# ohjay/snn-modulation-classification

Hardware: AMD Instinct MI355X
Metric: IQ windows/sec (RadioML 2x128, T=128) (higher is better)
Workload: dtype f32

## Files before the change

snn_modulation_classification_amd/csrc/dcll_hip.hip:

```cpp
#include "dcll_internal.h"

static thread_local char g_err[DCLL_ERR_LEN] = "";
char *dcll_err_buf(void) { return g_err; }

extern "C" int dcll_version(void) { return DCLL_ABI_VERSION; }
extern "C" const char *dcll_last_error(void) { return g_err; }

constexpr size_t DCLL_TRACE_LEN = 1 << 16;
static thread_local bool g_trace_on = false;
static thread_local size_t g_trace_len = 0;
static thread_local char *g_trace = nullptr;
void dcll_trace_note(const char *name)
{
    if (!g_trace_on || !g_trace) return;
    const size_t n = strlen(name);
    if (g_trace_len + n + 5 >= DCLL_TRACE_LEN) {
        if (g_trace_len + 4 < DCLL_TRACE_LEN && (g_trace_len < 4 || memcmp(g_trace + g_trace_len - 4, "...\n", 4) != 0)) {
            memcpy(g_trace + g_trace_len, "...\n", 4);
            g_trace_len += 4;
        }
        return;
    }
    memcpy(g_trace + g_trace_len, name, n);
    g_trace[g_trace_len + n] = '\n';
// ... 1251 lines not shown
            if (NRO > 0) {
                constexpr int RO_CH = (NRO > 24) ? 6 : 12;
                const f32x4 *wp = (const f32x4 *)ro_Wp + (long)((me * 4 + wq) * NRO) * 64 + lane;
#pragma unroll
                for (int n0 = 0; n0 < NRO; n0 += RO_CH) {
                    f32x4 wb[RO_CH];
#pragma unroll
                    for (int k = 0; k < RO_CH; ++k) wb[k] = wp[(n0 + k) * 64];
                    __builtin_amdgcn_sched_barrier(0);
#pragma unroll
                    for (int k = 0; k < RO_CH; ++k)
                        racc[n0 + k] = __builtin_fmaf(pvq[0], wb[k][0], __builtin_fmaf(pvq[1], wb[k][1],
                                       __builtin_fmaf(pvq[2], wb[k][2], __builtin_fmaf(pvq[3], wb[k][3], racc[n0 + k]))));
                    __builtin_amdgcn_sched_barrier(0);
                }
                if ((me >> 1) == 3) {
                    float *dst = ropart + ((te & 1) * NWAVE + w) * NRO;
#pragma unroll
                    for (int n = 0; n < NRO; ++n) {
                        const float tot = wave_sum_to_lane63(racc[n]);
                        if (lane == 63) dst[n] = tot;
                        racc[n] = 0.0f;
                    }
                }
            }
        }
        if (NRO > 0) {
            const int gc = g - 16;
            if (gc >= 0 && (gc & 7) == 0 && (gc >> 3) < T && w == ((gc >> 3) & 7) && lane < NRO) {
                const int tc = gc >> 3;
                const float *src = ropart + ((tc & 1) * NWAVE) * NRO + lane;
                float tot = ro_b[lane];
#pragma unroll
                for (int k = 0; k < NWAVE; ++k) tot += src[k * NRO];
                ro_out[((long)tc * B + b) * NRO + lane] = tot;
            }
        }
        if (ABLATE & 8) { unsigned long long x_ = __builtin_amdgcn_s_memtime(); dbg_epi += x_ - dbg_a; dbg_a = x_; }
        const int q = g - w;
        const bool active = q >= 0 && q < 8 * T;
        const bool tracing = active && !(ABLATE & 2) && (((q & 7) & 1) == tpar) && (q >> 3) + 1 < T;
        if (loaded && !tracing && !(PRIO & 4)) __builtin_amdgcn_s_setprio(0);
        if (active) {
            const int m = q & 7, t = q >> 3;
            float *img = lds + (t & 1) * IMG_FLOATS;
            if (tracing) {
                const int c = m >> 1;
                const float ta = tau4[0 * 32 + 4 * w + c], tm = tau4[1 * 32 + 4 * w + c];
                const float tas = tau4[2 * 32 + 4 * w + c], ts = tau4[3 * 32 + 4 * w + c];
                const unsigned long long w0 = pw0, w1 = pw1, w2 = pw2, w3 = pw3;
                {
                    const int tn = (c < 3) ? t + 1 : t + 2, cn = (c + 1) & 3;
                    if (tn < T) {
                        const unsigned long long *ip = in_wave + (long)tn * in_step + cn * 4;
                        pw0 = ip[0]; pw1 = ip[1]; pw2 = ip[2]; pw3 = ip[3];
                    }
                }
                const float *src = img + ioff + c * CHF;
                float *dst = lds + ((t + 1) & 1) * IMG_FLOATS + ioff + c * CHF;
                const float s0 = src[0], s1 = src[4 * ROWF], s2 = src[8 * ROWF], s3 = src[12 * ROWF];
                switch (c) {
#define DCLL_TRACE_CASE(C)                                                                \
    case C:                                                                               \
        trace_elem(w0, e0[C * 4 + 0], s0, dst + 0 * 4 * ROWF, ta, tm, tas, ts);           \
        trace_elem(w1, e0[C * 4 + 1], s1, dst + 1 * 4 * ROWF, ta, tm, tas, ts);           \
        trace_elem(w2, e0[C * 4 + 2], s2, dst + 2 * 4 * ROWF, ta, tm, tas, ts);           \
        trace_elem(w3, e0[C * 4 + 3], s3, dst + 3 * 4 * ROWF, ta, tm, tas, ts);           \
        break;
                    DCLL_TRACE_CASE(0)
                    DCLL_TRACE_CASE(1)
                    DCLL_TRACE_CASE(2)
                    DCLL_TRACE_CASE(3)
#undef DCLL_TRACE_CASE
                }
            }
            if (ABLATE & 8) { unsigned long long x_ = __builtin_amdgcn_s_memtime(); dbg_tr += x_ - dbg_a; dbg_a = x_; }
            if (loaded && tracing && !(PRIO & 4)) __builtin_amdgcn_s_setprio(0);
            f32x16 acc;
            if (w == 0 || (ABLATE & 4)) {
#pragma unroll
                for (int r = 0; r < 16; ++r) acc[r] = sbias[(r & 3) + 8 * (r >> 2) + 4 * h];
            } else {
                const f32x4 *sp = (const f32x4 *)(slots + ((w - 1) * 2 + ((g - 1) & 1)) * SLOT_FLOATS) + lane;
#pragma unroll
                for (int c = 0; c < 4; ++c) {
                    f32x4 v4 = sp[c * 64];
                    acc[4 * c + 0] = v4[0]; acc[4 * c + 1] = v4[1]; acc[4 * c + 2] = v4[2]; acc[4 * c + 3] = v4[3];
                }
            }
            const int i0 = (t & 1) * IMG_FLOATS + bbase + m * 2 * ROWF;
            int i1 = i0 + 2 * CHF;
            if (BASES == 2) asm volatile("" : "+v"(i1));
            auto tapval = [&](int cp, int off) -> float { return (BASES == 2 && cp) ? lds[i1 + off] : lds[i0 + cp * 2 * CHF + off]; };
            float bq[2][7];
#pragma unroll
            for (int kx = 0; kx < 7; ++kx) bq[0][kx] = tapval(0, kx);
#pragma unroll
            for (int r = 0; r < 14; ++r) {
                if (r + 1 < 14) {
                    const int cpn = (r + 1) / 7, kyn = (r + 1) % 7;
#pragma unroll
                    for (int kx = 0; kx < 7; ++kx) bq[(r + 1) & 1][kx] = tapval(cpn, kyn * ROWF + kx);
                }
                __builtin_amdgcn_sched_barrier(0);
#pragma unroll
                for (int kx = 0; kx < 7; ++kx)
                    acc = __builtin_amdgcn_mfma_f32_32x32x2f32(wf[r / 7][(r % 7) * 7 + kx], bq[r & 1][kx], acc, 0, 0, 0);
                __builtin_amdgcn_sched_barrier(0);
            }
            f32x4 *dp = (f32x4 *)(slots + (w * 2 + (g & 1)) * SLOT_FLOATS) + lane;
            if (ABLATE & 4) {
                if (acc[0] + acc[5] + acc[10] + acc[15] == 12345.678f) dp[0] = f32x4{acc[0], acc[1], acc[2], acc[3]};
            } else {
#pragma unroll
                for (int c = 0; c < 4; ++c) {
                    f32x4 v4 = {acc[4 * c + 0], acc[4 * c + 1], acc[4 * c + 2], acc[4 * c + 3]};
                    dp[c * 64] = v4;
                }
            }
        }
        if (loaded && (PRIO & 4)) __builtin_amdgcn_s_setprio(0);
        if (ABLATE & 8) {
            asm volatile("s_waitcnt vmcnt(0) lgkmcnt(0)" ::: "memory");
            unsigned long long x_ = __builtin_amdgcn_s_memtime();
            dbg_mf += x_ - dbg_a;
            __syncthreads();
            dbg_wait += __builtin_amdgcn_s_memtime() - x_;
        } else {
            __syncthreads();
        }
    }
    if ((ABLATE & 8) && lane == 0 && b == 0) {
        unsigned long long tot = __builtin_amdgcn_s_memtime() - dbg_t0;
        unsigned long long *dp = (unsigned long long *)v_out + w * 8;
        dp[0] = tot; dp[1] = dbg_wait; dp[2] = dbg_epi; dp[3] = dbg_tr; dp[4] = dbg_mf;
    }

    const float *fin = lds + ((T - 1) & 1) * IMG_FLOATS;
#pragma unroll
    for (int i = 0; i < 16; ++i) {
        long gidx = (b * 32 + 4 * w + (i >> 2)) * 256 + (i & 3) * 64 + lane;
        eps0_g[gidx] = e0[i];
        eps1_g[gidx] = fin[ioff + (i >> 2) * CHF + (i & 3) * 4 * ROWF];
    }
    if (REFRACTORY) {
#pragma unroll
        for (int k = 0; k < 4; ++k)
#pragma unroll
            for (int rr = 0; rr < 4; ++rr)
                arp_g[(b * 32 + rr + 8 * wq + 4 * h) * 256 + 32 * (2 * k + wpar) + j] = arp[k][rr];
    }
}

template <bool REFRACTORY, int OUT, int DBG = 0>
__global__ __launch_bounds__(512) void k_lif_seq_c32d(const uint32_t *__restrict__ spk_in, const dcll_wsrc W,
                                                       const float *__restrict__ bias, const float *__restrict__ tau4,
                                                       float *__restrict__ eps0_g, float *__restrict__ eps1_g,
                                                       float *__restrict__ arp_g, uint32_t *__restrict__ spk_out,
                                                       float *__restrict__ pv_out, float *__restrict__ v_out, int T,
                                                       int B, float alpharp, float wrp)
{
    __shared__ __attribute__((aligned(16))) float lds[2 * IMG_FLOATS + (NWAVE * 2 + 1) * SLOT_FLOATS];
    float *slots = lds + 2 * IMG_FLOATS;
    float *sbias = slots + NWAVE * 2 * SLOT_FLOATS;
    const int tid = threadIdx.x, lane = tid & 63, h = lane >> 5, j = lane & 31;
    const int wi = __builtin_amdgcn_readfirstlane(tid >> 6);
    const int w = (DBG & 4) ? wi : ((wi & 1) | ((wi & 4) >> 1) | ((wi & 2) << 1));
    const int wq = w & 3, wpar = w >> 2;
    const long b = blockIdx.x;
    __builtin_amdgcn_s_setprio(3);

    for (int i = tid; i < 2 * IMG_FLOATS; i += 512) lds[i] = 0.0f;
    for (int i = tid; i < SLOT_FLOATS; i += 512) sbias[i] = bias[(i & 3) + 8 * (i >> 8) + 4 * ((i >> 7) & 1)];

    float wf[2][49];
    load_wf_c32(W, j, w, h, wf);

    float e0[4][4];
    const int ioff = (4 * w) * CHF + ((lane >> 4) + 3) * ROWF + (lane & 15) + 3;
    const unsigned long long *in_wave = (const unsigned long long *)(spk_in + (b * 32 + 4 * w) * 8);
    const long in_step = (long)B * 32 * 4;
    __syncthreads();

#pragma unroll
    for (int grp = 0; grp < 4; ++grp) {
        const int c = (grp - w) & 3;
        const float ta = tau4[0 * 32 + 4 * w + c], tm = tau4[1 * 32 + 4 * w + c];
        const float tas = tau4[2 * 32 + 4 * w + c], ts = tau4[3 * 32 + 4 * w + c];
#pragma unroll
        for (int ii = 0; ii < 4; ++ii) {
            const long gidx = (b * 32 + 4 * w + c) * 256 + ii * 64 + lane;
            e0[grp][ii] = eps0_g[gidx];
            float e1 = eps1_g[gidx];
            float xin = (float)((in_wave[c * 4 + ii] >> lane) & 1ull);
            trace_update(xin, ta, tm, tas, ts, e0[grp][ii], e1);
            lds[ioff + c * CHF + ii * 4 * ROWF] = e1;
        }
    }
    float arp[4][4];
#pragma unroll
    for (int k = 0; k < 4; ++k)
#pragma unroll
        for (int rr = 0; rr < 4; ++rr)
            arp[k][rr] = REFRACTORY ? arp_g[(b * 32 + rr + 8 * wq + 4 * h) * 256 + 32 * (2 * k + wpar) + j] : 0.0f;

    const int bbase = (4 * w + h) * CHF + (j >> 4) * ((DBG & 2) ? 16 : ROWF) + (j & 15);
    const unsigned eoff = 4u * (4 * h * 256 + 32 * wpar + j);
#pragma unroll
    for (int k = 0; k < 4; ++k)
#pragma unroll
        for (int rr = 0; rr < 4; ++rr) asm volatile("" ::"v"(arp[k][rr]));
#pragma unroll
    for (int grp = 0; grp < 4; ++grp)
#pragma unroll
        for (int ii = 0; ii < 4; ++ii) asm volatile("" ::"v"(e0[grp][ii]));
#pragma unroll
    for (int cp = 0; cp < 2; ++cp)
#pragma unroll
        for (int k = 0; k < 49; ++k) asm volatile("" ::"v"(wf[cp][k]));
    __syncthreads();

    unsigned long long dbg[4] = {0, 0, 0, 0}, dbg_t0 = 0;
    if (DBG & 1) dbg_t0 = __builtin_amdgcn_s_memtime();
    float sv[4] = {0.f, 0.f, 0.f, 0.f}, ta = 0.f, tm = 0.f, tas = 0.f, ts = 0.f;
    unsigned long long wm[4] = {0, 0, 0, 0};
    auto fetch_trace_inputs = [&](const int g) {
        const int q = g - w;
        if (q >= 0 && q < 4 * T && (q >> 2) + 1 < T) {
            const int p = q & 3, t = q >> 2;
            const float *src = lds + (t & 1) * IMG_FLOATS + ioff + p * CHF;
#pragma unroll
            for (int i = 0; i < 4; ++i) sv[i] = src[i * 4 * ROWF];
            const unsigned long long *ip = in_wave + (long)(t + 1) * in_step + p * 4;
#pragma unroll
            for (int i = 0; i < 4; ++i) wm[i] = ip[i];
            ta = tau4[0 * 32 + 4 * w + p]; tm = tau4[1 * 32 + 4 * w + p];
            tas = tau4[2 * 32 + 4 * w + p]; ts = tau4[3 * 32 + 4 * w + p];
        }
    };
    fetch_trace_inputs(0);
    auto stage = [&](const int g, auto UC) {
        constexpr int U = decltype(UC)::value;
        unsigned long long st0 = 0, st1 = 0, st2 = 0, st3 = 0;
        if (DBG & 1) st0 = __builtin_amdgcn_s_memtime();
        const int q = g - w;
        const bool active = q >= 0 && q < 4 * T;
        const int p = q & 3, t = q >> 2;
        f32x16 accA, accB;
        if (active) {
            const float *inA = (w == 0) ? sbias : slots + ((w - 1) * 2) * SLOT_FLOATS;
            const float *inB = (w == 0) ? sbias : slots + ((w - 1) * 2 + 1) * SLOT_FLOATS;
            const f32x4 *spa = (const f32x4 *)inA + lane, *spb = (const f32x4 *)inB + lane;
#pragma unroll
            for (int c = 0; c < 4; ++c) {
                f32x4 va = spa[c * 64], vb = spb[c * 64];
                accA[4 * c + 0] = va[0]; accA[4 * c + 1] = va[1]; accA[4 * c + 2] = va[2]; accA[4 * c + 3] = va[3];
                accB[4 * c + 0] = vb[0]; accB[4 * c + 1] = vb[1]; accB[4 * c + 2] = vb[2]; accB[4 * c + 3] = vb[3];
            }
        }
        const int qe = g - 8;
        const bool epi = qe >= 0 && qe < 4 * T;
        f32x4 v4 = {0.f, 0.f, 0.f, 0.f};
        if (epi) v4 = *((const f32x4 *)(slots + (7 * 2 + wpar) * SLOT_FLOATS) + wq * 64 + lane);
        const bool tr = active && t + 1 < T;
        const int i0 = (t & 1) * IMG_FLOATS + bbase + p * 4 * ROWF;
        const bool skip = !(DBG & 4);
        const int rl = (skip && p == 0) ? 2 : 0;
        lds_cfloat *ib0 = (lds_cfloat *)(lds + i0), *ib1 = (lds_cfloat *)(lds + i0 + 2 * CHF);
        asm volatile("" : "+v"(ib0), "+v"(ib1));
        float bq[2][7];
        if (active) {
#pragma unroll
            for (int kx = 0; kx < 7; ++kx) bq[0][kx] = ib0[rl * ROWF + kx];
        }
        if (tr) {
            float *dst = lds + ((t + 1) & 1) * IMG_FLOATS + ioff + p * CHF;
#pragma unroll
            for (int i = 0; i < 4; ++i) {
                float a;
                asm("v_cndmask_b32 %0, 0, %1, %2" : "=v"(a) : "v"(ts), "s"(wm[i]));
                const float bb = tas * e0[U][i];
                e0[U][i] = a + bb;
                const float cc = ta * sv[i];
                const float dd = e0[U][i] * tm;
                dst[i * 4 * ROWF] = cc + dd;
            }
        }
        if (epi) {
            const int te = qe >> 2, me = 2 * U + wpar;
            const long ubase = (((long)te * B + b) * 32 + 8 * wq) * 256;
            const auto prs = tile_rsrc(pv_out + ubase), vrs = tile_rsrc(v_out + ubase);
            uint32_t myword = 0;
#pragma unroll
            for (int rr = 0; rr < 4; ++rr) {
                float v = v4[rr];
                bool s;
                if (REFRACTORY) v = refractory(v4[rr], arp[U][rr], alpharp, wrp, s);
                else s = v > 0.0f;
                const unsigned long long mk = __ballot(s);
                const uint32_t mine = h ? (uint32_t)(mk >> 32) : (uint32_t)mk;
                myword = (j == rr) ? mine : myword;
                if (OUT & 1) __builtin_amdgcn_raw_buffer_store_b32(__float_as_uint(sigmoidf_dev(v)), prs, eoff + 4u * (rr * 256 + 64 * U), 0, 0);
                if (OUT & 2) __builtin_amdgcn_raw_buffer_store_b32(__float_as_uint(v), vrs, eoff + 4u * (rr * 256 + 64 * U), 0, 0);
            }
            if (spk_out && j < 4)
                __builtin_amdgcn_raw_buffer_store_b32(myword, tile_rsrc(spk_out + (ubase >> 5)), 4u * ((4 * h + j) * 8 + wpar) + 8u * U, 0, 0);
        }
        if (DBG & 1) { asm volatile("s_waitcnt lgkmcnt(0)" ::: "memory"); st1 = __builtin_amdgcn_s_memtime(); }
        lds_barrier();
        if (DBG & 1) st2 = __builtin_amdgcn_s_memtime();
        fetch_trace_inputs(g + 1);
        if (active) {
            auto chains = [&](auto RLC, auto RHC) {
                constexpr int RL = decltype(RLC)::value, RH = decltype(RHC)::value, NRH = RH - RL, NR = 2 * NRH;
#pragma unroll
                for (int r = 0; r < NR; ++r) {
                    const int cp = r / NRH, rho = RL + r % NRH;
                    if (r + 1 < NR) {
                        const int cpn = (r + 1) / NRH, rhon = RL + (r + 1) % NRH;
#pragma unroll
                        for (int kx = 0; kx < 7; ++kx) bq[(r + 1) & 1][kx] = (cpn ? ib1 : ib0)[rhon * ROWF + kx];
                    }
                    __builtin_amdgcn_sched_barrier(0);
#pragma unroll
                    for (int kx = 0; kx < 7; ++kx) {
                        if (rho <= 6)
                            accA = __builtin_amdgcn_mfma_f32_32x32x2f32(wf[cp][rho * 7 + kx], bq[r & 1][kx], accA, 0, 0, 0);
                        if (rho >= 2)
                            accB = __builtin_amdgcn_mfma_f32_32x32x2f32(wf[cp][(rho - 2) * 7 + kx], bq[r & 1][kx], accB, 0, 0, 0);
                    }
                    __builtin_amdgcn_sched_barrier(0);
                    if (cp == 1 && rho == 6 && r + 1 < NR) {
                        f32x4 *dpa = (f32x4 *)(slots + (w * 2) * SLOT_FLOATS) + lane;
#pragma unroll
                        for (int c = 0; c < 4; ++c)
                            dpa[c * 64] = f32x4{accA[4 * c + 0], accA[4 * c + 1], accA[4 * c + 2], accA[4 * c + 3]};
                        __builtin_amdgcn_sched_barrier(0);
                    }
                }
                if (RH == 7) {
                    f32x4 *dpa = (f32x4 *)(slots + (w * 2) * SLOT_FLOATS) + lane;
#pragma unroll
                    for (int c = 0; c < 4; ++c)
                        dpa[c * 64] = f32x4{accA[4 * c + 0], accA[4 * c + 1], accA[4 * c + 2], accA[4 * c + 3]};
                }
            };
            if (skip && p == 0) chains(std::integral_constant<int, 2>{}, std::integral_constant<int, 9>{});
            else if (skip && p == 3) chains(std::integral_constant<int, 0>{}, std::integral_constant<int, 7>{});
            else chains(std::integral_constant<int, 0>{}, std::integral_constant<int, 9>{});
            f32x4 *dp = (f32x4 *)(slots + (w * 2 + 1) * SLOT_FLOATS) + lane;
#pragma unroll
            for (int c = 0; c < 4; ++c)
                dp[c * 64] = f32x4{accB[4 * c + 0], accB[4 * c + 1], accB[4 * c + 2], accB[4 * c + 3]};
        }
        if (DBG & 1) { asm volatile("s_waitcnt lgkmcnt(0)" ::: "memory"); st3 = __builtin_amdgcn_s_memtime(); }
        lds_barrier();
        if (DBG & 1) {
            const unsigned long long st4 = __builtin_amdgcn_s_memtime();
            dbg[0] += st1 - st0; dbg[1] += st2 - st1; dbg[2] += st3 - st2; dbg[3] += st4 - st3;
        }
    };

    const int nstage = 4 * T + 8;
    for (int g = 0; g < nstage; g += 4) {
        stage(g + 0, std::integral_constant<int, 0>{});
        stage(g + 1, std::integral_constant<int, 1>{});
        stage(g + 2, std::integral_constant<int, 2>{});
        stage(g + 3, std::integral_constant<int, 3>{});
    }

    if ((DBG & 1) && lane == 0 && b == 0) {
        unsigned long long *dp = (unsigned long long *)v_out + w * 8;
        dp[0] = __builtin_amdgcn_s_memtime() - dbg_t0;
        dp[1] = dbg[0]; dp[2] = dbg[1]; dp[3] = dbg[2]; dp[4] = dbg[3];
    }
    const float *fin = lds + ((T - 1) & 1) * IMG_FLOATS;
#pragma unroll
    for (int grp = 0; grp < 4; ++grp) {
        const int c = (grp - w) & 3;
#pragma unroll
        for (int ii = 0; ii < 4; ++ii) {
            const long gidx = (b * 32 + 4 * w + c) * 256 + ii * 64 + lane;
            eps0_g[gidx] = e0[grp][ii];
            eps1_g[gidx] = fin[ioff + c * CHF + ii * 4 * ROWF];
        }
    }
    if (REFRACTORY) {
#pragma unroll
        for (int k = 0; k < 4; ++k)
#pragma unroll
            for (int rr = 0; rr < 4; ++rr)
                arp_g[(b * 32 + rr + 8 * wq + 4 * h) * 256 + 32 * (2 * k + wpar) + j] = arp[k][rr];
    }
}

__global__ void k_permute_readout(const float *__restrict__ Wt, float *__restrict__ Wp, int N)
{
    int i = blockIdx.x * blockDim.x + threadIdx.x;
    if (i >= N * 8192) return;
    int rr = i & 3, lane = (i >> 2) & 63;
    int r = i >> 8;
    int n = r % N;
    r /= N;
    int wq = r & 3, me = r >> 2;
    int co = rr + 8 * wq + 4 * (lane >> 5), pix = 32 * me + (lane & 31);
    Wp[i] = Wt[(long)n * 8192 + co * 256 + pix];
}

static inline unsigned nblk(long n, int bs) { return (unsigned)((n + bs - 1) / bs); }

static int launch_readout(const float *pv, const float *Wt, const float *bias, float *out, long rows, int K, int N,
                          hipStream_t st, int mode = DCLL_READOUT_AUTO)
{
    if (rows == 0 || N == 0) return DCLL_OK;
    const bool fast = (K % RO_KC == 0) && N <= 64 && (((uintptr_t)pv | (uintptr_t)Wt) & 15) == 0 &&
                      K < (1 << 22);
    const bool direct_ok = fast && K % 64 == 0 && N <= 48 && K <= 16384 && mode != DCLL_READOUT_LDS;
    if (direct_ok && mode == DCLL_READOUT_CORESIDENT)
        return dcll_launch_readout_direct(pv, Wt, bias, out, rows, K, N, st);
    if (fast && mode == DCLL_READOUT_T16) return dcll_launch_readout_t16(pv, Wt, bias, out, rows, K, N, 0, st);
    if (rows <= 2048) {
        hipLaunchKernelGGL(k_readout_rows, dim3((unsigned)((rows + RS_RB - 1) / RS_RB), (N + RS_NG - 1) / RS_NG), dim3(256),
                           0, st, pv, Wt, bias, out, rows, K, N);
    } else if (fast && K % RK_KC == 0 && K >= 65536 && rows < 256L * RO_ROWS) {
        if (N <= 32)
            hipLaunchKernelGGL(k_readout_ks<1>, dim3(nblk(rows, RK_ROWS)), dim3(256), 0, st, pv, Wt, bias, out, rows, K, N, 0);
        else
            hipLaunchKernelGGL(k_readout_ks<2>, dim3(nblk(rows, RK_ROWS)), dim3(256), 0, st, pv, Wt, bias, out, rows, K, N, 0);
    } else if (fast && mode != DCLL_READOUT_LDS) {
        return dcll_launch_readout_t16(pv, Wt, bias, out, rows, K, N, 0, st);
    } else if (fast && N <= 32) {
        hipLaunchKernelGGL(k_readout_v4<1>, dim3(nblk(rows, RO_ROWS)), dim3(256), 0, st, pv, Wt, bias, out, rows, K, N);
    } else if (fast) {
        hipLaunchKernelGGL(k_readout_v4<2>, dim3(nblk(rows, RO_ROWS)), dim3(256), 0, st, pv, Wt, bias, out, rows, K, N);
    } else {
        dim3 grid(nblk(rows, RO_ROWS), (N + 31) / 32);
        hipLaunchKernelGGL(k_readout, grid, dim3(256), 0, st, pv, Wt, bias, out, rows, K, N);
    }
    HIP_CHECK_LAUNCH("k_readout");
    return DCLL_OK;
}

extern "C" int dcll_readout(const float *pv, const float *Wt, const float *bias, float *out, int64_t rows, int32_t K,
                            int32_t N, void *stream)
{
    if (rows == 0) return DCLL_OK;
    if (!pv || !Wt || !out || rows < 0 || K < 1 || N < 1) return fail(DCLL_ERR_INVALID, "dcll_readout: bad argument");
    return launch_readout(pv, Wt, bias, out, rows, K, N, (hipStream_t)stream);
}

extern "C" int dcll_readout_mode(const float *pv, const float *Wt, const float *bias, float *out, int64_t rows,
                                 int32_t K, int32_t N, int32_t mode, void *stream)
{
    if (rows == 0) return DCLL_OK;
    if (!pv || !Wt || !out || rows < 0 || K < 1 || N < 1 || mode < DCLL_READOUT_AUTO || mode > DCLL_READOUT_T16)
        return fail(DCLL_ERR_INVALID, "dcll_readout_mode: bad argument");
    return launch_readout(pv, Wt, bias, out, rows, K, N, (hipStream_t)stream, mode);
}

__global__ __launch_bounds__(256) void k_readout_sum(const float *__restrict__ part, const float *__restrict__ bias,
                                                      float *__restrict__ out, long n_out, int N, int nslice)
{
    __shared__ float red[4][64];
    const long i = (long)blockIdx.x * 64 + (threadIdx.x & 63);
    const int grp = threadIdx.x >> 6;
    float acc = 0.0f;
    if (i < n_out) {
        const int per = (nslice + 3) / 4, s0 = grp * per, s1 = min(nslice, s0 + per);
        for (int sl = s0; sl < s1; ++sl) acc += part[(long)sl * n_out + i];
    }
    red[grp][threadIdx.x & 63] = acc;
    __syncthreads();
    if (grp == 0 && i < n_out) {
        const int l = threadIdx.x & 63;
        out[i] = (bias ? bias[i % N] : 0.0f) + (((red[0][l] + red[1][l]) + red[2][l]) + red[3][l]);
    }
}

static int splitk_slice(int64_t rows, int32_t K, int32_t N)
{
    if (rows < 1 || N < 1 || N > 64) return 0;
    if (K >= 65536 && K % 4096 == 0) {
        return rows <= 2048 ? 4096 : K / 8;
    }
    if (rows <= 2048 && K >= 2048 && K < 65536 && K % 256 == 0) return (rows <= 512 && N <= 32) ? 128 : 256;
    return 0;
}

extern "C" int64_t dcll_readout_splitk_scratch(int64_t rows, int32_t K, int32_t N)
{
    const int ks = splitk_slice(rows, K, N);
    return ks ? (int64_t)(K / ks) * rows * N : 0;
}

extern "C" int dcll_readout_splitk(const float *pv, const float *Wt, const float *bias, float *out, float *scratch,
                                   int64_t scratch_floats, int64_t rows, int32_t K, int32_t N, void *stream)
{
    if (rows == 0 || N == 0) return DCLL_OK;
    if (!pv || !Wt || !out || !scratch || rows < 0 || K < 1 || N < 1)
        return fail(DCLL_ERR_INVALID, "dcll_readout_splitk: bad argument");
    const int ks = splitk_slice(rows, K, N);
    if (ks == 0 || ((((uintptr_t)pv | (uintptr_t)Wt)) & 15) != 0)
        return fail(DCLL_ERR_UNSUPPORTED, "dcll_readout_splitk: needs N <= 64, 16-byte aligned operands and K >= 65536 with "
                                          "K % 4096 == 0, or rows <= 2048 with 2048 <= K < 65536, K % 256 == 0");
    if (scratch_floats < dcll_readout_splitk_scratch(rows, K, N))
        return fail(DCLL_ERR_INVALID, "dcll_readout_splitk: scratch too small (dcll_readout_splitk_scratch)");
    hipStream_t st = (hipStream_t)stream;
    const int nslice = K / ks;
    if (ks != 4096) {
        int rc = dcll_launch_readout_t16(pv, Wt, nullptr, scratch, rows, K, N, ks, st);
        if (rc) return rc;
    } else {
        dim3 grid(nblk(rows, RK_ROWS), nslice);
        if (N <= 32) hipLaunchKernelGGL(k_readout_ks<1>, grid, dim3(256), 0, st, pv, Wt, bias, scratch, rows, K, N, 4096);
        else hipLaunchKernelGGL(k_readout_ks<2>, grid, dim3(256), 0, st, pv, Wt, bias, scratch, rows, K, N, 4096);
        HIP_CHECK_LAUNCH("k_readout_ks (split K)");
    }
    hipLaunchKernelGGL(k_readout_sum, dim3(nblk(rows * N, 64)), dim3(256), 0, st, scratch, bias, out, rows * N, N, nslice);
    HIP_CHECK_LAUNCH("k_readout_sum");
    return DCLL_OK;
}

static int act_nslice(int32_t K)
{
    if (K < 65536 || K % 256 != 0) return 0;
    int n = 8;
    while (n < 64 && K / (2 * n) >= 8192 && K % (2 * n * RO_KC) == 0) n *= 2;
    return n;
}
extern "C" int64_t dcll_readout_act_scratch(int64_t rows, int32_t K, int32_t N)
{
    return (rows > 0 && N > 0) ? (int64_t)act_nslice(K) * rows * N : 0;
}

extern "C" int dcll_readout_act(const float *pv, const float *Wt, const float *bias, float *out, float *scratch,
                                int64_t scratch_floats, int64_t rows, int32_t K, int32_t N, int32_t act, void *stream)
{
    if (rows == 0 || N == 0) return DCLL_OK;
    if (!pv || !Wt || !out || rows < 0 || K < 1 || N < 1 || (act != DCLL_ACT_NONE && act != DCLL_ACT_SIGMOID))
        return fail(DCLL_ERR_INVALID, "dcll_readout_act: bad argument");
    if (!(K % RO_KC == 0 && K < (1 << 22) && N <= 64 && (((uintptr_t)pv | (uintptr_t)Wt) & 15) == 0))
        return fail(DCLL_ERR_UNSUPPORTED, "dcll_readout_act: needs K % 32 == 0, K < 2^22, N <= 64, 16-byte aligned pv / Wt");
    hipStream_t st = (hipStream_t)stream;
    const int64_t need = dcll_readout_act_scratch(rows, K, N);
    if (need == 0) return dcll_launch_readout_t16(pv, Wt, bias, out, rows, K, N, 0, st, act);
// ... 1417 lines not shown
```

Measured before the change: 20650.

## Switch fused LIF conv kernel from 32x32x2 to 16x16x4 MFMA tiling

Rewrites the sequential LIF convolution stage to use v_mfma_f32_16x16x4f32 instead of 32x32x2. This changes the weight-fragment layout, the accumulator layout, the bias and epilogue indexing, and the spike-word packing. A compile-time schedule of 56 steps skips taps that fall outside the image and shares B-operand loads between the low and high accumulator chains. The stage loop is no longer unrolled by four, which shrinks code size. A standalone probe checks that the 16x16 MFMA accumulates in the same order as a forward fmaf chain, so results stay bit-exact. The risk is different MFMA throughput and issue density, plus extra LDS address registers.

```diff
diff --git a/experiments/mfma16_order_probe.hip b/experiments/mfma16_order_probe.hip
--- /dev/null
+++ b/experiments/mfma16_order_probe.hip
@@ -0,0 +1,83 @@
+#include <hip/hip_runtime.h>
+#include <math.h>
+#include <stdio.h>
+#include <stdlib.h>
+#include <string.h>
+#include <vector>
+typedef float f32x4 __attribute__((ext_vector_type(4)));
+
+__global__ __launch_bounds__(256) void k_probe(const float *a, const float *b, const float *c, float *d, int nwave)
+{
+    const int wv = blockIdx.x * 4 + (threadIdx.x >> 6), lane = threadIdx.x & 63;
+    if (wv >= nwave) return;
+    const long o = (long)wv * 64 + lane;
+    f32x4 acc;
+    for (int r = 0; r < 4; ++r) acc[r] = c[o * 4 + r];
+    acc = __builtin_amdgcn_mfma_f32_16x16x4f32(a[o], b[o], acc, 0, 0, 0);
+    for (int r = 0; r < 4; ++r) d[o * 4 + r] = acc[r];
+}
+
+static float rnd(unsigned long long &s)
+{
+    s = s * 6364136223846793005ull + 1442695040888963407ull;
+    const double u = (double)(s >> 11) / 9007199254740992.0;
+    s = s * 6364136223846793005ull + 1442695040888963407ull;
+    const int e = (int)((s >> 33) % 49) - 24;
+    s = s * 6364136223846793005ull + 1442695040888963407ull;
+    const float sg = (s >> 40) & 1 ? -1.0f : 1.0f;
+    return sg * ldexpf((float)(1.0 + u), e);
+}
+
+#define CK(x) do { hipError_t e_ = (x); if (e_ != hipSuccess) { printf("%s: %s\n", #x, hipGetErrorString(e_)); return 2; } } while (0)
+
+int main()
+{
+    const int NW = 4096;
+    std::vector<float> a(NW * 64), b(NW * 64), c(NW * 256), d(NW * 256);
+    unsigned long long s = 12345;
+    for (auto &x : a) x = rnd(s);
+    for (auto &x : b) x = rnd(s);
+    for (int w = 0; w < NW; ++w)
+        for (int l = 0; l < 64; ++l)
+            for (int r = 0; r < 4; ++r) {
+                const int i = 4 * (l >> 4) + r, j = l & 15;
+                const float p = a[w * 64 + i] * b[w * 64 + j];
+                c[(w * 64 + l) * 4 + r] = -p * (1.0f + ldexpf(rnd(s) > 0.0f ? 1.0f : -1.0f, -12 - (int)(s % 8)));
+            }
+    float *da, *db, *dc, *dd;
+    CK(hipMalloc(&da, a.size() * 4)); CK(hipMalloc(&db, b.size() * 4));
+    CK(hipMalloc(&dc, c.size() * 4)); CK(hipMalloc(&dd, d.size() * 4));
+    CK(hipMemcpy(da, a.data(), a.size() * 4, hipMemcpyHostToDevice));
+    CK(hipMemcpy(db, b.data(), b.size() * 4, hipMemcpyHostToDevice));
+    CK(hipMemcpy(dc, c.data(), c.size() * 4, hipMemcpyHostToDevice));
+    hipLaunchKernelGGL(k_probe, dim3(NW / 4), dim3(256), 0, 0, da, db, dc, dd, NW);
+    CK(hipGetLastError());
+    CK(hipDeviceSynchronize());
+    CK(hipMemcpy(d.data(), dd, d.size() * 4, hipMemcpyDeviceToHost));
+    long bad_fwd = 0, bad_rev = 0, bad_exact = 0, bad_pair = 0, n = 0;
+    for (int w = 0; w < NW; ++w)
+        for (int l = 0; l < 64; ++l)
+            for (int r = 0; r < 4; ++r) {
+                const int i = 4 * (l >> 4) + r, j = l & 15;
+                float A[4], Bv[4];
+                for (int k = 0; k < 4; ++k) { A[k] = a[w * 64 + i + 16 * k]; Bv[k] = b[w * 64 + j + 16 * k]; }
+                const float C = c[(w * 64 + l) * 4 + r], D = d[(w * 64 + l) * 4 + r];
+                float fwd = C, rev = C;
+                for (int k = 0; k < 4; ++k) fwd = fmaf(A[k], Bv[k], fwd);
+                for (int k = 3; k >= 0; --k) rev = fmaf(A[k], Bv[k], rev);
+                double ex = C;
+                for (int k = 0; k < 4; ++k) ex += (double)A[k] * Bv[k];
+                const float pair = C + (fmaf(A[1], Bv[1], A[0] * Bv[0]) + fmaf(A[3], Bv[3], A[2] * Bv[2]));
+                bad_fwd += memcmp(&fwd, &D, 4) != 0;
+                bad_rev += memcmp(&rev, &D, 4) != 0;
+                bad_exact += (float)ex != D;
+                bad_pair += memcmp(&pair, &D, 4) != 0;
+                ++n;
+            }
+    printf("v_mfma_f32_16x16x4_f32, %ld results: differ from the forward fmaf chain k = 0..3: %ld; reverse chain: %ld; "
+           "exact sum rounded once: %ld; pairwise: %ld\n", n, bad_fwd, bad_rev, bad_exact, bad_pair);
+    const bool ok = bad_fwd == 0 && bad_rev > 0 && bad_pair > 0;
+    printf("%s\n", ok ? "ORDER OK (forward chain, bit for bit; the data separates the other orders)" : "ORDER MISMATCH");
+    hipFree(da); hipFree(db); hipFree(dc); hipFree(dd);
+    return ok ? 0 : 1;
+}
diff --git a/snn_modulation_classification_amd/csrc/dcll_hip.hip b/snn_modulation_classification_amd/csrc/dcll_hip.hip
--- a/snn_modulation_classification_amd/csrc/dcll_hip.hip
+++ b/snn_modulation_classification_amd/csrc/dcll_hip.hip
@@ -1427,6 +1427,49 @@
     }
 }
 
+constexpr int c16_cp(int t2) { return t2 / 49; }
+constexpr int c16_ky(int t2) { return (t2 % 49) / 7; }
+constexpr int c16_kx(int t2) { return t2 % 7; }
+constexpr int c16_base(int i) { return i == 24 ? 4 : (c16_kx(2 * i) == 6 ? 2 : 0) + c16_cp(2 * i); }
+constexpr int c16_imm(int rl, int i) { return (rl + c16_ky(2 * i)) * ROWF + c16_kx(2 * i); }
+constexpr bool c16_run(int V, int rl, int i)
+{
+    const int y = (V == 1 ? 0 : V == 2 ? 12 : 4) + rl;
+    for (int dk = 0; dk < 2; ++dk) {
+        const int yy = y + c16_ky(2 * i + dk) - 3;
+        if (yy >= 0 && yy < 16) return true;
+    }
+    return false;
+}
+constexpr bool c16_lo(int V, int P, int s) { return s <= 48 && c16_run(V, P, s); }
+constexpr bool c16_hi(int V, int P, int s) { return s >= 7 && c16_run(V, P + 2, s - 7); }
+constexpr bool c16_shared(int V, int P, int s)
+{
+    return c16_lo(V, P, s) && c16_hi(V, P, s) && c16_base(s) == c16_base(s - 7) && c16_imm(P, s) == c16_imm(P + 2, s - 7);
+}
+constexpr int C16_STEPS = 56, C16_PD = 1;
+
+__device__ __forceinline__ void load_wf_c16(const dcll_wsrc &W, int lane, int w, float (&wf)[2][49])
+{
+    const int co = lane & 15, dk = lane >> 5;
+    const long r0 = ((long)co * 32 + 4 * w + ((lane >> 4) & 1)) * 49 + dk, r1 = r0 + 16L * 32 * 49, x24 = 49 * dk;
+    auto off = [&](int i) -> long { return 2 * i + (i > 24 ? 49 : 0) + (i == 24 ? x24 : 0); };
+    if (W.q) {
+        const float s0 = W.scale[co], s1 = W.scale[16 + co];
+#pragma unroll
+        for (int i = 0; i < 49; ++i) {
+            wf[0][i] = (float)W.q[r0 + off(i)] * s0;
+            wf[1][i] = (float)W.q[r1 + off(i)] * s1;
+        }
+    } else {
+#pragma unroll
+        for (int i = 0; i < 49; ++i) {
+            wf[0][i] = W.f[r0 + off(i)];
+            wf[1][i] = W.f[r1 + off(i)];
+        }
+    }
+}
+
 template <bool REFRACTORY, int OUT, int DBG = 0>
 __global__ __launch_bounds__(512) void k_lif_seq_c32d(const uint32_t *__restrict__ spk_in, const dcll_wsrc W,
                                                        const float *__restrict__ bias, const float *__restrict__ tau4,
@@ -1438,18 +1481,19 @@
     __shared__ __attribute__((aligned(16))) float lds[2 * IMG_FLOATS + (NWAVE * 2 + 1) * SLOT_FLOATS];
     float *slots = lds + 2 * IMG_FLOATS;
     float *sbias = slots + NWAVE * 2 * SLOT_FLOATS;
-    const int tid = threadIdx.x, lane = tid & 63, h = lane >> 5, j = lane & 31;
+    const int tid = threadIdx.x, lane = tid & 63;
     const int wi = __builtin_amdgcn_readfirstlane(tid >> 6);
     const int w = (DBG & 4) ? wi : ((wi & 1) | ((wi & 4) >> 1) | ((wi & 2) << 1));
-    const int wq = w & 3, wpar = w >> 2;
+    const int es = w >> 2, eh = w & 1, er = (w >> 1) & 1;
+    const int eco = 16 * eh + 4 * (lane >> 4) + 2 * er, epx = 32 * es + (lane & 15);
     const long b = blockIdx.x;
     __builtin_amdgcn_s_setprio(3);
 
     for (int i = tid; i < 2 * IMG_FLOATS; i += 512) lds[i] = 0.0f;
-    for (int i = tid; i < SLOT_FLOATS; i += 512) sbias[i] = bias[(i & 3) + 8 * (i >> 8) + 4 * ((i >> 7) & 1)];
+    for (int i = tid; i < SLOT_FLOATS; i += 512) sbias[i] = bias[16 * ((i >> 8) & 1) + 4 * ((i >> 6) & 3) + (i & 3)];
 
     float wf[2][49];
-    load_wf_c32(W, j, w, h, wf);
+    load_wf_c16(W, lane, w, wf);
 
     float e0[4][4];
     const int ioff = (4 * w) * CHF + ((lane >> 4) + 3) * ROWF + (lane & 15) + 3;
@@ -1476,11 +1520,13 @@
 #pragma unroll
     for (int k = 0; k < 4; ++k)
 #pragma unroll
-        for (int rr = 0; rr < 4; ++rr)
-            arp[k][rr] = REFRACTORY ? arp_g[(b * 32 + rr + 8 * wq + 4 * h) * 256 + 32 * (2 * k + wpar) + j] : 0.0f;
-
-    const int bbase = (4 * w + h) * CHF + (j >> 4) * ((DBG & 2) ? 16 : ROWF) + (j & 15);
-    const unsigned eoff = 4u * (4 * h * 256 + 32 * wpar + j);
+        for (int rl = 0; rl < 2; ++rl)
+#pragma unroll
+            for (int rr = 0; rr < 2; ++rr)
+                arp[k][2 * rl + rr] = REFRACTORY ? arp_g[(b * 32 + eco + rr) * 256 + 64 * k + 16 * rl + epx] : 0.0f;
+
+    const int bl = (4 * w + ((lane >> 4) & 1)) * CHF + (lane & 15), bdk = lane >> 5;
+    const unsigned eoff = 4u * (eco * 256 + epx);
 #pragma unroll
     for (int k = 0; k < 4; ++k)
 #pragma unroll
@@ -1490,9 +1536,9 @@
 #pragma unroll
         for (int ii = 0; ii < 4; ++ii) asm volatile("" ::"v"(e0[grp][ii]));
 #pragma unroll
-    for (int cp = 0; cp < 2; ++cp)
-#pragma unroll
-        for (int k = 0; k < 49; ++k) asm volatile("" ::"v"(wf[cp][k]));
+    for (int hf = 0; hf < 2; ++hf)
+#pragma unroll
+        for (int k = 0; k < 49; ++k) asm volatile("" ::"v"(wf[hf][k]));
     __syncthreads();
 
     unsigned long long dbg[4] = {0, 0, 0, 0}, dbg_t0 = 0;
@@ -1514,40 +1560,9 @@
         }
     };
     fetch_trace_inputs(0);
-    auto stage = [&](const int g, auto UC) {
+
+    auto nonmfma = [&](const int g, const bool tr, const int p, const int t, const f32x2 (&ev)[2], auto UC) {
         constexpr int U = decltype(UC)::value;
-        unsigned long long st0 = 0, st1 = 0, st2 = 0, st3 = 0;
-        if (DBG & 1) st0 = __builtin_amdgcn_s_memtime();
-        const int q = g - w;
-        const bool active = q >= 0 && q < 4 * T;
-        const int p = q & 3, t = q >> 2;
-        f32x16 accA, accB;
-        if (active) {
-            const float *inA = (w == 0) ? sbias : slots + ((w - 1) * 2) * SLOT_FLOATS;
-            const float *inB = (w == 0) ? sbias : slots + ((w - 1) * 2 + 1) * SLOT_FLOATS;
-            const f32x4 *spa = (const f32x4 *)inA + lane, *spb = (const f32x4 *)inB + lane;
-#pragma unroll
-            for (int c = 0; c < 4; ++c) {
-                f32x4 va = spa[c * 64], vb = spb[c * 64];
-                accA[4 * c + 0] = va[0]; accA[4 * c + 1] = va[1]; accA[4 * c + 2] = va[2]; accA[4 * c + 3] = va[3];
-                accB[4 * c + 0] = vb[0]; accB[4 * c + 1] = vb[1]; accB[4 * c + 2] = vb[2]; accB[4 * c + 3] = vb[3];
-            }
-        }
-        const int qe = g - 8;
-        const bool epi = qe >= 0 && qe < 4 * T;
-        f32x4 v4 = {0.f, 0.f, 0.f, 0.f};
-        if (epi) v4 = *((const f32x4 *)(slots + (7 * 2 + wpar) * SLOT_FLOATS) + wq * 64 + lane);
-        const bool tr = active && t + 1 < T;
-        const int i0 = (t & 1) * IMG_FLOATS + bbase + p * 4 * ROWF;
-        const bool skip = !(DBG & 4);
-        const int rl = (skip && p == 0) ? 2 : 0;
-        lds_cfloat *ib0 = (lds_cfloat *)(lds + i0), *ib1 = (lds_cfloat *)(lds + i0 + 2 * CHF);
-        asm volatile("" : "+v"(ib0), "+v"(ib1));
-        float bq[2][7];
-        if (active) {
-#pragma unroll
-            for (int kx = 0; kx < 7; ++kx) bq[0][kx] = ib0[rl * ROWF + kx];
-        }
         if (tr) {
             float *dst = lds + ((t + 1) & 1) * IMG_FLOATS + ioff + p * CHF;
 #pragma unroll
@@ -1561,72 +1576,135 @@
                 dst[i * 4 * ROWF] = cc + dd;
             }
         }
-        if (epi) {
-            const int te = qe >> 2, me = 2 * U + wpar;
-            const long ubase = (((long)te * B + b) * 32 + 8 * wq) * 256;
+        const int qe = g - 8;
+        if (qe >= 0 && qe < 4 * T) {
+            const int te = qe >> 2;
+            const long ubase = ((long)te * B + b) * 32 * 256;
             const auto prs = tile_rsrc(pv_out + ubase), vrs = tile_rsrc(v_out + ubase);
-            uint32_t myword = 0;
-#pragma unroll
-            for (int rr = 0; rr < 4; ++rr) {
-                float v = v4[rr];
-                bool s;
-                if (REFRACTORY) v = refractory(v4[rr], arp[U][rr], alpharp, wrp, s);
-                else s = v > 0.0f;
-                const unsigned long long mk = __ballot(s);
-                const uint32_t mine = h ? (uint32_t)(mk >> 32) : (uint32_t)mk;
-                myword = (j == rr) ? mine : myword;
-                if (OUT & 1) __builtin_amdgcn_raw_buffer_store_b32(__float_as_uint(sigmoidf_dev(v)), prs, eoff + 4u * (rr * 256 + 64 * U), 0, 0);
-                if (OUT & 2) __builtin_amdgcn_raw_buffer_store_b32(__float_as_uint(v), vrs, eoff + 4u * (rr * 256 + 64 * U), 0, 0);
-            }
-            if (spk_out && j < 4)
-                __builtin_amdgcn_raw_buffer_store_b32(myword, tile_rsrc(spk_out + (ubase >> 5)), 4u * ((4 * h + j) * 8 + wpar) + 8u * U, 0, 0);
+            unsigned long long mk[2][2];
+#pragma unroll
+            for (int rl = 0; rl < 2; ++rl)
+#pragma unroll
+                for (int rr = 0; rr < 2; ++rr) {
+                    float v = ev[rl][rr];
+                    bool s;
+                    if (REFRACTORY) v = refractory(ev[rl][rr], arp[U][2 * rl + rr], alpharp, wrp, s);
+                    else s = v > 0.0f;
+                    mk[rl][rr] = __ballot(s);
+                    const unsigned imm = 4u * (rr * 256 + 16 * rl + 64 * U);
+                    if (OUT & 1) __builtin_amdgcn_raw_buffer_store_b32(__float_as_uint(sigmoidf_dev(v)), prs, eoff + imm, 0, 0);
+                    if (OUT & 2) __builtin_amdgcn_raw_buffer_store_b32(__float_as_uint(v), vrs, eoff + imm, 0, 0);
+                }
+            if (spk_out && lane < 8) {
+                const int sh = 16 * (lane >> 1);
+                const unsigned long long m0 = (lane & 1) ? mk[0][1] : mk[0][0], m1 = (lane & 1) ? mk[1][1] : mk[1][0];
+                const uint32_t word = ((uint32_t)(m0 >> sh) & 0xffffu) | ((uint32_t)(m1 >> sh) << 16);
+                const unsigned woff = 4u * ((16 * eh + 4 * (lane >> 1) + 2 * er + (lane & 1)) * 8 + es);
+                __builtin_amdgcn_raw_buffer_store_b32(word, tile_rsrc(spk_out + (ubase >> 5)), woff + 8u * U, 0, 0);
+            }
+        }
+    };
+
+    auto stage = [&](const int g) {
+        unsigned long long st0 = 0, st1 = 0, st2 = 0, st3 = 0;
+        if (DBG & 1) st0 = __builtin_amdgcn_s_memtime();
+        const int q = g - w;
+        const bool active = q >= 0 && q < 4 * T;
+        const int p = q & 3, t = q >> 2;
+        f32x4 acc[4][2];
+        if (active) {
+            const float *inA = (w == 0) ? sbias : slots + ((w - 1) * 2) * SLOT_FLOATS;
+            const float *inB = (w == 0) ? sbias : slots + ((w - 1) * 2 + 1) * SLOT_FLOATS;
+            const f32x4 *spa = (const f32x4 *)inA + lane, *spb = (const f32x4 *)inB + lane;
+#pragma unroll
+            for (int rl = 0; rl < 2; ++rl)
+#pragma unroll
+                for (int hf = 0; hf < 2; ++hf) {
+                    acc[rl][hf] = spa[(2 * rl + hf) * 64];
+                    acc[2 + rl][hf] = spb[(2 * rl + hf) * 64];
+                }
+        }
+        const int qe = g - 8;
+        f32x2 ev[2] = {{0.f, 0.f}, {0.f, 0.f}};
+        if (qe >= 0 && qe < 4 * T) {
+            const f32x2 *ep = (const f32x2 *)(slots + (7 * 2 + es) * SLOT_FLOATS) + 2 * lane + er;
+            ev[0] = ep[(0 + eh) * 128];
+            ev[1] = ep[(2 + eh) * 128];
+        }
+        const int i0 = (t & 1) * IMG_FLOATS + bl + p * 4 * ROWF;
+        lds_cfloat *bs[5] = {(lds_cfloat *)(lds + i0 + bdk), (lds_cfloat *)(lds + i0 + 2 * CHF + bdk),
+                             (lds_cfloat *)(lds + i0 + bdk * (ROWF - 6)), (lds_cfloat *)(lds + i0 + 2 * CHF + bdk * (ROWF - 6)),
+                             (lds_cfloat *)(lds + i0 + bdk * (2 * CHF - 6 * ROWF - 6))};
+        asm volatile("" : "+v"(bs[0]), "+v"(bs[1]), "+v"(bs[2]), "+v"(bs[3]), "+v"(bs[4]));
+        const int V = (DBG & 4) ? 0 : p == 0 ? 1 : p == 3 ? 2 : 0;
+        float bv[C16_PD + 1][4];
+        auto load = [&](auto VC, auto SC) {
+            constexpr int Vc = decltype(VC)::value, s = decltype(SC)::value;
+            static_for<0, 2>([&](auto PC) {
+                constexpr int P = decltype(PC)::value;
+                if constexpr (c16_lo(Vc, P, s)) bv[s % (C16_PD + 1)][2 * P] = bs[c16_base(s)][c16_imm(P, s)];
+                if constexpr (c16_hi(Vc, P, s) && !c16_shared(Vc, P, s)) {
+                    constexpr int i = s >= 7 ? s - 7 : 0;
+                    bv[s % (C16_PD + 1)][2 * P + 1] = bs[c16_base(i)][c16_imm(P + 2, i)];
+                }
+            });
+        };
+        if (active) {
+            if (V == 1) static_for<0, C16_PD>([&](auto SC) { load(std::integral_constant<int, 1>{}, SC); });
+            else if (V == 2) static_for<0, C16_PD>([&](auto SC) { load(std::integral_constant<int, 2>{}, SC); });
+            else static_for<0, C16_PD>([&](auto SC) { load(std::integral_constant<int, 0>{}, SC); });
+        }
+        const bool tr = active && t + 1 < T;
+        switch (g & 3) {
+        case 0: nonmfma(g, tr, p, t, ev, std::integral_constant<int, 0>{}); break;
+        case 1: nonmfma(g, tr, p, t, ev, std::integral_constant<int, 1>{}); break;
+        case 2: nonmfma(g, tr, p, t, ev, std::integral_constant<int, 2>{}); break;
+        default: nonmfma(g, tr, p, t, ev, std::integral_constant<int, 3>{}); break;
         }
         if (DBG & 1) { asm volatile("s_waitcnt lgkmcnt(0)" ::: "memory"); st1 = __builtin_amdgcn_s_memtime(); }
         lds_barrier();
         if (DBG & 1) st2 = __builtin_amdgcn_s_memtime();
         fetch_trace_inputs(g + 1);
         if (active) {
-            auto chains = [&](auto RLC, auto RHC) {
-                constexpr int RL = decltype(RLC)::value, RH = decltype(RHC)::value, NRH = RH - RL, NR = 2 * NRH;
-#pragma unroll
-                for (int r = 0; r < NR; ++r) {
-                    const int cp = r / NRH, rho = RL + r % NRH;
-                    if (r + 1 < NR) {
-                        const int cpn = (r + 1) / NRH, rhon = RL + (r + 1) % NRH;
-#pragma unroll
-                        for (int kx = 0; kx < 7; ++kx) bq[(r + 1) & 1][kx] = (cpn ? ib1 : ib0)[rhon * ROWF + kx];
-                    }
+            f32x4 *dp = (f32x4 *)(slots + (w * 2) * SLOT_FLOATS) + lane;
+            auto chains = [&](auto VC) {
+                constexpr int Vc = decltype(VC)::value;
+                static_for<0, C16_STEPS>([&](auto SC) {
+                    constexpr int s = decltype(SC)::value, nb = s % (C16_PD + 1);
+                    constexpr int il = s <= 48 ? s : 48, ih = s >= 7 ? s - 7 : 0;
+                    if constexpr (s + C16_PD < C16_STEPS) load(VC, std::integral_constant<int, s + C16_PD>{});
                     __builtin_amdgcn_sched_barrier(0);
-#pragma unroll
-                    for (int kx = 0; kx < 7; ++kx) {
-                        if (rho <= 6)
-                            accA = __builtin_amdgcn_mfma_f32_32x32x2f32(wf[cp][rho * 7 + kx], bq[r & 1][kx], accA, 0, 0, 0);
-                        if (rho >= 2)
-                            accB = __builtin_amdgcn_mfma_f32_32x32x2f32(wf[cp][(rho - 2) * 7 + kx], bq[r & 1][kx], accB, 0, 0, 0);
-                    }
+                    static_for<0, 2>([&](auto PC) {
+                        constexpr int P = decltype(PC)::value;
+                        if constexpr (c16_lo(Vc, P, s)) {
+                            acc[P][0] = __builtin_amdgcn_mfma_f32_16x16x4f32(wf[0][il], bv[nb][2 * P], acc[P][0], 0, 0, 0);
+                            acc[P][1] = __builtin_amdgcn_mfma_f32_16x16x4f32(wf[1][il], bv[nb][2 * P], acc[P][1], 0, 0, 0);
+                        }
+                    });
+                    static_for<0, 2>([&](auto PC) {
+                        constexpr int P = decltype(PC)::value, bi = c16_shared(Vc, P, s) ? 2 * P : 2 * P + 1;
+                        if constexpr (c16_hi(Vc, P, s)) {
+                            acc[P + 2][0] = __builtin_amdgcn_mfma_f32_16x16x4f32(wf[0][ih], bv[nb][bi], acc[P + 2][0], 0, 0, 0);
+                            acc[P + 2][1] = __builtin_amdgcn_mfma_f32_16x16x4f32(wf[1][ih], bv[nb][bi], acc[P + 2][1], 0, 0, 0);
+                        }
+                    });
                     __builtin_amdgcn_sched_barrier(0);
-                    if (cp == 1 && rho == 6 && r + 1 < NR) {
-                        f32x4 *dpa = (f32x4 *)(slots + (w * 2) * SLOT_FLOATS) + lane;
-#pragma unroll
-                        for (int c = 0; c < 4; ++c)
-                            dpa[c * 64] = f32x4{accA[4 * c + 0], accA[4 * c + 1], accA[4 * c + 2], accA[4 * c + 3]};
+                    if constexpr (s == 49) {
+#pragma unroll
+                        for (int rl = 0; rl < 2; ++rl)
+#pragma unroll
+                            for (int hf = 0; hf < 2; ++hf) dp[(2 * rl + hf) * 64] = acc[rl][hf];
                         __builtin_amdgcn_sched_barrier(0);
                     }
-                }
-                if (RH == 7) {
-                    f32x4 *dpa = (f32x4 *)(slots + (w * 2) * SLOT_FLOATS) + lane;
-#pragma unroll
-                    for (int c = 0; c < 4; ++c)
-                        dpa[c * 64] = f32x4{accA[4 * c + 0], accA[4 * c + 1], accA[4 * c + 2], accA[4 * c + 3]};
-                }
+                });
             };
-            if (skip && p == 0) chains(std::integral_constant<int, 2>{}, std::integral_constant<int, 9>{});
-            else if (skip && p == 3) chains(std::integral_constant<int, 0>{}, std::integral_constant<int, 7>{});
-            else chains(std::integral_constant<int, 0>{}, std::integral_constant<int, 9>{});
-            f32x4 *dp = (f32x4 *)(slots + (w * 2 + 1) * SLOT_FLOATS) + lane;
-#pragma unroll
-            for (int c = 0; c < 4; ++c)
-                dp[c * 64] = f32x4{accB[4 * c + 0], accB[4 * c + 1], accB[4 * c + 2], accB[4 * c + 3]};
+            if (V == 1) chains(std::integral_constant<int, 1>{});
+            else if (V == 2) chains(std::integral_constant<int, 2>{});
+            else chains(std::integral_constant<int, 0>{});
+#pragma unroll
+            for (int rl = 0; rl < 2; ++rl)
+#pragma unroll
+                for (int hf = 0; hf < 2; ++hf) dp[SLOT_FLOATS / 4 + (2 * rl + hf) * 64] = acc[2 + rl][hf];
         }
         if (DBG & 1) { asm volatile("s_waitcnt lgkmcnt(0)" ::: "memory"); st3 = __builtin_amdgcn_s_memtime(); }
         lds_barrier();
@@ -1637,12 +1715,8 @@
     };
 
     const int nstage = 4 * T + 8;
-    for (int g = 0; g < nstage; g += 4) {
-        stage(g + 0, std::integral_constant<int, 0>{});
-        stage(g + 1, std::integral_constant<int, 1>{});
-        stage(g + 2, std::integral_constant<int, 2>{});
-        stage(g + 3, std::integral_constant<int, 3>{});
-    }
+#pragma clang loop unroll(disable)
+    for (int g = 0; g < nstage; ++g) stage(g);
 
     if ((DBG & 1) && lane == 0 && b == 0) {
         unsigned long long *dp = (unsigned long long *)v_out + w * 8;
@@ -1664,8 +1738,10 @@
 #pragma unroll
         for (int k = 0; k < 4; ++k)
 #pragma unroll
-            for (int rr = 0; rr < 4; ++rr)
-                arp_g[(b * 32 + rr + 8 * wq + 4 * h) * 256 + 32 * (2 * k + wpar) + j] = arp[k][rr];
+            for (int rl = 0; rl < 2; ++rl)
+#pragma unroll
+                for (int rr = 0; rr < 2; ++rr)
+                    arp_g[(b * 32 + eco + rr) * 256 + 64 * k + 16 * rl + epx] = arp[k][2 * rl + rr];
     }
 }
 
```

New measurement: 20800 (median of 6 runs). Within noise of the previous version (+0.7%).
